# sergree/matchering

Measured on NVIDIA H100. Metric: stereo 44.1kHz samples/sec (x real-time), higher is better.
Workload: dtype f32

## Files before the change

matchering_b200/csrc/limiter.cu:

```cuda
#include <math.h>
#include <string.h>

#include "kernels.cuh"

namespace mgb {

namespace {

constexpr int NT = kLimiterThreads;
constexpr int CORE_EPT = kLimiterCoreEpt;
constexpr int LC = kLimiterCore;
constexpr int SPAN_EPT_MAX = kLimiterSpanEptMax;

__device__ __forceinline__ double scan_carry(double B, const ScanPow* t, double c0, double* scratch) {
    const int lane = threadIdx.x & 31, warp = threadIdx.x >> 5;
    double v = B;
#pragma unroll
    for (int d = 1; d < 32; d <<= 1) {
        const double up = __shfl_up_sync(0xffffffffu, v, d);
        if (lane >= d) v += t->ql[d] * up;
    }
    if (lane == 31) scratch[warp] = v;
    __syncthreads();
    double w = lane < NT / 32 ? scratch[lane] : 0.0;
#pragma unroll
    for (int d = 1; d < NT / 32; d <<= 1) {
        const double up = __shfl_up_sync(0xffffffffu, w, d);
        if (lane >= d) w += t->qw[d] * up;
    }
    const double warp_carry = __shfl_sync(0xffffffffu, w, (warp + 31) & 31);
    double prev = __shfl_up_sync(0xffffffffu, v, 1);
    if (lane == 0) prev = 0.0;
    return prev + t->ql[lane] * ((warp > 0 ? warp_carry : 0.0) + t->qw[warp] * c0);
}

__device__ __forceinline__ double scan_carry_rev(double B, const ScanPow* t, const double* c0, double* scratch) {
    const int lane = threadIdx.x & 31, warp = threadIdx.x >> 5;
    const int rl = 31 - lane, rw = NT / 32 - 1 - warp;
    double v = B;
#pragma unroll
    for (int d = 1; d < 32; d <<= 1) {
        const double up = __shfl_down_sync(0xffffffffu, v, d);
        if (rl >= d) v += t->ql[d] * up;
    }
    if (lane == 0) scratch[rw] = v;
    __syncthreads();
    double w = lane < NT / 32 ? scratch[lane] : 0.0;
#pragma unroll
    for (int d = 1; d < NT / 32; d <<= 1) {
        const double up = __shfl_up_sync(0xffffffffu, w, d);
        if (lane >= d) w += t->qw[d] * up;
    }
    const double warp_carry = __shfl_sync(0xffffffffu, w, (rw + 31) & 31);
    double prev = __shfl_down_sync(0xffffffffu, v, 1);
    if (rl == 0) prev = 0.0;
    return prev + t->ql[rl] * ((rw > 0 ? warp_carry : 0.0) + t->qw[rw] * (*c0));
}

template <int N>
struct StVec {
    double v[N];
};
template <int N>
__device__ __forceinline__ StVec<N> st_zero() {
    StVec<N> z;
#pragma unroll
    for (int i = 0; i < N; ++i) z.v[i] = 0.0;
    return z;
}
template <int N>
__device__ __forceinline__ StVec<N> st_shfl_up(StVec<N> a, int d) {
#pragma unroll
    for (int i = 0; i < N; ++i) a.v[i] = __shfl_up_sync(0xffffffffu, a.v[i], d);
    return a;
}
template <int N>
__device__ __forceinline__ StVec<N> st_shfl(StVec<N> a, int src) {
#pragma unroll
    for (int i = 0; i < N; ++i) a.v[i] = __shfl_sync(0xffffffffu, a.v[i], src);
    return a;
}
template <int N>
__device__ __forceinline__ void st_addmul(StVec<N>& y, const double (*M)[N], const StVec<N>& x) {
#pragma unroll
    for (int r = 0; r < N; ++r)
#pragma unroll
        for (int c = 0; c < N; ++c) y.v[r] += M[r][c] * x.v[c];
}
template <int N>
__device__ __forceinline__ StVec<N> st_mul(const double (*M)[N], const StVec<N>& x) {
    StVec<N> y = st_zero<N>();
    st_addmul<N>(y, M, x);
    return y;
}

template <int N>
__device__ __forceinline__ StVec<N> section_scan(StVec<N> B, const SectionTab<N>* t, double* scratch) {
    const int lane = threadIdx.x & 31, warp = threadIdx.x >> 5;
    StVec<N> v = B;
#pragma unroll
    for (int d = 1; d < 32; d <<= 1) {
        const StVec<N> up = st_shfl_up<N>(v, d);
        if (lane >= d) st_addmul<N>(v, t->ql[d], up);
    }
    if (lane == 31) {
#pragma unroll
        for (int i = 0; i < N; ++i) scratch[warp * N + i] = v.v[i];
    }
    __syncthreads();
    StVec<N> w = st_zero<N>();
    if (lane < NT / 32) {
#pragma unroll
        for (int i = 0; i < N; ++i) w.v[i] = scratch[lane * N + i];
    }
#pragma unroll
    for (int d = 1; d < NT / 32; d <<= 1) {
        const StVec<N> up = st_shfl_up<N>(w, d);
        if (lane >= d) st_addmul<N>(w, t->qw[d], up);
    }
    StVec<N> warp_carry = st_shfl<N>(w, (warp + 31) & 31);
    if (warp == 0) warp_carry = st_zero<N>();
    StVec<N> prev = st_shfl_up<N>(v, 1);
    if (lane == 0) prev = st_zero<N>();
    st_addmul<N>(prev, t->ql[lane], warp_carry);
    return prev;
}

template <int N>
__device__ __forceinline__ StVec<N> section_lead(const SectionTab<N>* t, const StVec<N>& cin) {
    const int lane = threadIdx.x & 31, warp = threadIdx.x >> 5;
    return st_mul<N>(t->ql[lane], st_mul<N>(t->qw[warp], cin));
}

__device__ __forceinline__ void publish(LookbackWord* w, double v, int status) {
#ifdef MGB_EMULATE
    w->value = v;
    w->status = status;
#else
    asm volatile("st.global.cg.v2.u64 [%0], {%1, %2};" ::"l"(w), "l"(__double_as_longlong(v)), "l"((long long)status) : "memory");
#endif
}
__device__ __forceinline__ int poll(const LookbackWord* w, double* v) {
#ifdef MGB_EMULATE
    *v = w->value;
    return (int)w->status;
#else
    long long a, b;
    asm volatile("ld.global.cg.v2.u64 {%0, %1}, [%2];" : "=l"(a), "=l"(b) : "l"(w) : "memory");
    *v = __longlong_as_double(a);
    return (int)b;
#endif
}

template <int N>
__device__ __forceinline__ StVec<N> lookback(const LookbackWord* words , int chunk,
                                             const SectionTab<N>* t) {
    constexpr int STRIDE = 2 * N;
    const int lane = threadIdx.x & 31;
    if constexpr (N == 1) {
        double acc1 = 0.0, m1 = 1.0;
        for (int base = chunk - 1; base >= 0 && m1 > 1e-9; base -= 32) {
            const int j = base - lane;
            int st = 2;
            double val = 0.0;
            if (j >= 0) {
                const LookbackWord* w = words + (long long)j * STRIDE;
                while ((st = poll(w, &val)) == 0) __nanosleep(20);
            }
            const unsigned inclusive = __ballot_sync(0xffffffffu, st == 2);
            const int first = inclusive ? __ffs((int)inclusive) - 1 : 32;
            if (lane <= first) acc1 += m1 * t->pc[lane][0][0] * val;
            if (inclusive) break;
            m1 *= t->pc[32][0][0];
        }
        StVec<N> out;
        out.v[0] = warp_sum(acc1);
        return out;
    }
    StVec<N> acc = st_zero<N>();
    double mult[N][N];
    int jump = 0;
    for (int base = chunk - 1; base >= 0; base -= 32, ++jump) {
        if (N > 1 && jump < kLookbackJumps) {
#pragma unroll
            for (int r = 0; r < N; ++r)
#pragma unroll
                for (int c = 0; c < N; ++c) mult[r][c] = t->pj[jump][r][c];
        } else if (jump == 0) {
#pragma unroll
            for (int r = 0; r < N; ++r)
#pragma unroll
                for (int c = 0; c < N; ++c) mult[r][c] = r == c ? 1.0 : 0.0;
        } else {
            double next[N][N];
#pragma unroll
            for (int r = 0; r < N; ++r)
#pragma unroll
                for (int c = 0; c < N; ++c) {
                    double sum = 0.0;
#pragma unroll
                    for (int k = 0; k < N; ++k) sum += mult[r][k] * t->pc[32][k][c];
                    next[r][c] = sum;
                }
#pragma unroll
            for (int r = 0; r < N; ++r)
#pragma unroll
                for (int c = 0; c < N; ++c) mult[r][c] = next[r][c];
        }
        double bound = 0.0;
#pragma unroll
        for (int r = 0; r < N; ++r) {
            double rowsum = 0.0;
#pragma unroll
            for (int c = 0; c < N; ++c) rowsum += fabs(mult[r][c]);
            bound = fmax(bound, rowsum);
        }
        if (bound <= 1e-9) break;
        const int j = base - lane;
        int st = 2;
        StVec<N> val = st_zero<N>();
        if (j >= 0) {
            const LookbackWord* w = words + (long long)j * STRIDE;
            for (;;) {
                st = poll(w, &val.v[0]);
                bool same = st != 0;
#pragma unroll
                for (int i = 1; i < N; ++i) same = same && poll(w + i, &val.v[i]) == st;
                if (same) break;
                __nanosleep(20);
            }
        }
        const unsigned inclusive = __ballot_sync(0xffffffffu, st == 2);
        const int first = inclusive ? __ffs((int)inclusive) - 1 : 32;
        if (lane <= first) st_addmul<N>(acc, mult, st_mul<N>(t->pc[lane], val));
        if (inclusive) break;
    }
#pragma unroll
    for (int i = 0; i < N; ++i) acc.v[i] = warp_sum(acc.v[i]);
    return acc;
}
template <int N>
__device__ __forceinline__ void publish_state(LookbackWord* words, const StVec<N>& s, int status) {
#pragma unroll
    for (int i = 0; i < N; ++i) publish(words + i, s.v[i], status);
}

struct LimiterGeom {
    int reach, hold, warm, left;
    int ept;
    int span;
    int filt;
    int publish_inclusive;
    int shared_core;
    int margin;
    int use_ticket;
};

__global__ void limiter_tables_kernel(mgb_limiter_params lp, int span_ept, unsigned char* tables) {
    const int i = threadIdx.x;
    ScanPow* att = reinterpret_cast<ScanPow*>(tables);
    {
        const double p = lp.attack_c;
        if (i < SPAN_EPT_MAX + 2) att->pe[i] = pow(p, (double)i);
        if (i < 33) att->ql[i] = pow(p, (double)(span_ept * i));
        if (i < 17) att->qw[i] = pow(p, (double)(span_ept * 32 * i));
        if (i < 33) att->pc[i] = pow(p, (double)LC * (double)i);
    }
    SectionTab<1>* sec = reinterpret_cast<SectionTab<1>*>(tables + sizeof(ScanPow));
    for (int f = 0; f < 2; ++f) {
        const double p = f == 0 ? -lp.hold_a[1] : -lp.release_a[1];
        SectionTab<1>* t = sec + f;
        if (i < CORE_EPT) t->pe[i][0] = pow(p, (double)(i + 1));
        if (i < 33) t->ql[i][0][0] = pow(p, (double)(CORE_EPT * i));
        if (i < 17) t->qw[i][0][0] = pow(p, (double)(CORE_EPT * 32 * i));
        if (i < 33) t->pc[i][0][0] = pow(p, (double)LC * (double)i);
        for (int j = i; j < kLookbackJumps; j += blockDim.x) t->pj[j][0][0] = pow(p, (double)LC * 32.0 * (double)j);
    }
}

template <int EPT, int NO, bool GAINS = false>
__global__ void __launch_bounds__(NT, (NO == 1 && EPT <= 17) ? 2 : 1)
limiter_kernel(mgb_limiter_params lp, LimiterGeom gm, const float2* __restrict__ in, float2* __restrict__ out,
               long long frames, const double* __restrict__ pre_gain, const double* __restrict__ post_gain,
               const int* __restrict__ engaged, int* __restrict__ ticket, LookbackWord* __restrict__ slots,
               const unsigned char* __restrict__ tables) {
    constexpr int HC = CORE_EPT + NO;
    constexpr int CAP = EPT * NT;
    MGB_DYN_SMEM(smem);
    double* Fd = reinterpret_cast<double*>(smem);
    float* Aenv = reinterpret_cast<float*>(smem) + CAP;
    float* G = reinterpret_cast<float*>(smem + (size_t)CAP * 8) + gm.margin;
    float* Wk = G + CAP + gm.margin;
    __shared__ float blockmax[NT];
    __shared__ ScanPow pw_att;
    __shared__ SectionTab<1> pw_sec[2];
    __shared__ double scratch_a[32 * NO], scratch_b[32 * NO];
    __shared__ double bcast[2 + 2 * NO];
    __shared__ int chunk_s;
    const ScanPow* pow_att = &pw_att;
    const SectionTab<NO>* sec_global = reinterpret_cast<const SectionTab<NO>*>(tables + sizeof(ScanPow));
    const SectionTab<NO>* tab_hold = NO == 1 ? reinterpret_cast<const SectionTab<NO>*>(&pw_sec[0]) : sec_global;
    const SectionTab<NO>* tab_rel = NO == 1 ? reinterpret_cast<const SectionTab<NO>*>(&pw_sec[1]) : sec_global + 1;

    const int tid = threadIdx.x;
    int chunk = blockIdx.x;
    if (gm.use_ticket) {
        if (tid == 0) chunk_s = atomicAdd(ticket, 1);
        __syncthreads();
        chunk = chunk_s;
    }
    const long long s0 = (long long)chunk * LC;
    const int core_n = (int)((s0 + LC < frames) ? LC : frames - s0);
    const int reach = gm.reach, hold = gm.hold, HL = gm.left, FL = gm.filt;
    const long long ga = s0 - HL - reach;
    const int cidx = HL + reach;
    const int vlo = ga < 0 ? (int)(-ga) : 0;
    const int vhi = (frames - ga < (long long)gm.span) ? (int)(frames - ga) : gm.span;
    const double thr = lp.threshold;

    float2 v[EPT];
    {
        const float2* base = in + ga;
#pragma unroll
        for (int k = 0; k < EPT; ++k) {
            const int i = tid + k * NT;
            v[k] = (i >= vlo && i < vhi) ? __ldg(base + i) : make_float2(0.0f, 0.0f);
        }
    }
    const double pre = pre_gain ? *pre_gain : 1.0;
    const double post = post_gain ? *post_gain : 1.0;
    const double scale = pre * post;
    const bool bypass = engaged && *engaged == 0;
    {
        const double* src = reinterpret_cast<const double*>(tables);
        double* dst = reinterpret_cast<double*>(&pw_att);
        for (int i = tid; i < (int)(sizeof(ScanPow) / sizeof(double)); i += NT) dst[i] = src[i];
        if (NO == 1) {
            src += sizeof(ScanPow) / sizeof(double);
            dst = reinterpret_cast<double*>(pw_sec);
            for (int i = tid; i < (int)(2 * sizeof(SectionTab<1>) / sizeof(double)); i += NT) dst[i] = src[i];
        }
    }
    if (bypass) {
        for (int k = tid; k < core_n; k += NT) {
            const float2 w = in[s0 + k];
            out[s0 + k] = make_float2((float)((double)w.x * pre * post), (float)((double)w.y * pre * post));
        }
        return;
    }
    for (int i = tid; i < gm.margin; i += NT) {
        G[-1 - i] = 0.0f;
        G[CAP + i] = 0.0f;
    }
#pragma unroll
    for (int k = 0; k < EPT; ++k) {
        const double a = (double)fmaxf(fabsf(v[k].x), fabsf(v[k].y)) * pre;
        const double over = a - thr;
        float g = 0.0f;
        if (over > 0.0) g = __fdiv_rn((float)over, (float)a);
        G[tid + k * NT] = g;
    }
    __syncthreads();

    float hc[HC];
    {
        float* PF = reinterpret_cast<float*>(smem);
        float* SF = Wk;
        float x[EPT];
        const int base = tid * EPT;
#pragma unroll
        for (int e = 0; e < EPT; ++e) x[e] = G[base + e];
        float run = 0.0f;
#pragma unroll
        for (int e = 0; e < EPT; ++e) {
            run = fmaxf(run, x[e]);
            PF[base + e] = run;
        }
        blockmax[tid] = run;
        run = 0.0f;
#pragma unroll
        for (int e = EPT - 1; e >= 0; --e) {
            run = fmaxf(run, x[e]);
            SF[base + e] = run;
        }
        __syncthreads();
        auto whole_blocks = [&](int a, int b) -> float {
            float m = 0.0f;
            for (int q = a; q <= b; ++q) m = fmaxf(m, blockmax[q]);
            return m;
        };
        auto window = [&](int l, int r, int br, float pr) -> float {
            const int bl = l / EPT;
            if (bl == br) {
                float m = 0.0f;
                for (int i = l; i <= r; ++i) m = fmaxf(m, G[i]);
                return m;
            }
            float m = fmaxf(SF[l], pr);
            if (br - bl > 1) m = fmaxf(m, whole_blocks(bl + 1, br - 1));
            return m;
        };
        auto gat = [&](int i) -> float { return G[i]; };
        if (gm.shared_core) {
            float la[EPT], rt[EPT];
#pragma unroll
            for (int e = 0; e < EPT - 1; ++e) {
                la[e] = gat(base - reach + e);
                rt[e + 1] = gat(base + reach + 1 + e);
            }
            la[EPT - 1] = rt[0] = 0.0f;
#pragma unroll
            for (int e = EPT - 2; e >= 0; --e) la[e] = fmaxf(la[e], la[e + 1]);
#pragma unroll
            for (int e = 1; e < EPT; ++e) rt[e] = fmaxf(rt[e], rt[e - 1]);
            const int r = min(base + reach, CAP - 1);
            const float core = window(max(base + EPT - 1 - reach, 0), r, r / EPT, PF[r]);
#pragma unroll
            for (int e = 0; e < EPT; ++e) Aenv[base + e] = fmaxf(core, fmaxf(la[e], rt[e]));
        } else {
#pragma unroll
            for (int e = 0; e < EPT; ++e) {
                const int i = base + e;
                const int r = min(i + reach, CAP - 1);
                Aenv[i] = window(max(i - reach, 0), r, r / EPT, PF[r]);
            }
        }
        const int bh = cidx + tid * CORE_EPT - NO;
        if (gm.shared_core) {
            float lh[HC], rh[HC];
#pragma unroll
            for (int e = 0; e < HC - 1; ++e) {
                lh[e] = gat(bh - reach - hold + 1 + e);
                rh[e + 1] = gat(bh + reach + 1 + e);
            }
            lh[HC - 1] = rh[0] = 0.0f;
#pragma unroll
            for (int e = HC - 2; e >= 0; --e) lh[e] = fmaxf(lh[e], lh[e + 1]);
#pragma unroll
            for (int e = 1; e < HC; ++e) rh[e] = fmaxf(rh[e], rh[e - 1]);
            const int r = min(bh + reach, CAP - 1);
            const float core = window(max(bh + HC - reach - hold, 0), r, r / EPT, PF[r]);
#pragma unroll
            for (int e = 0; e < HC; ++e) hc[e] = fmaxf(core, fmaxf(lh[e], rh[e]));
        } else {
#pragma unroll
            for (int e = 0; e < HC; ++e) {
                const int r = min(bh + e + reach, CAP - 1);
                hc[e] = window(max(bh + e - reach - hold + 1, 0), r, r / EPT, PF[r]);
            }
        }
#pragma unroll
        for (int e = 0; e < HC; ++e)
            if (bh + e < vlo) hc[e] = 0.0f;
    }

    LookbackWord* slot_hold = slots + (long long)chunk * (2 * NO);
    LookbackWord* slot_rel = slot_hold + NO;
    double hold_y[CORE_EPT];
    StVec<NO> hold_carry;
    float* Hown = Wk + tid * HC;
    {
#pragma unroll
        for (int e = 0; e < CORE_EPT; ++e) {
            double acc = lp.hold_b[0] * (double)hc[e + NO];
#pragma unroll
            for (int i = 1; i <= NO; ++i) acc += lp.hold_b[i] * (double)hc[e + NO - i];
#pragma unroll
            for (int i = 1; i <= NO; ++i)
                if (e - i >= 0) acc -= lp.hold_a[i] * hold_y[e - i];
            hold_y[e] = acc;
        }
        StVec<NO> end;
#pragma unroll
        for (int i = 0; i < NO; ++i) end.v[i] = hold_y[CORE_EPT - 1 - i];
        hold_carry = section_scan<NO>(end, tab_hold, scratch_a);
        if (tid == NT - 1) {
            st_addmul<NO>(end, tab_hold->ql[1], hold_carry);
            publish_state<NO>(slot_hold, end, 1);
        }
#pragma unroll
        for (int e = 0; e < HC; ++e) Hown[e] = hc[e];
    }

    const double c = lp.attack_c;
    const bool edge_l = vlo > reach, edge_r = vhi < reach + FL;
    if (edge_l || edge_r) {
        const int i0 = vlo, iL = vhi - 1;
        float fix[EPT];
#pragma unroll
        for (int k = 0; k < EPT; ++k) {
            const int i = tid + k * NT;
            fix[k] = Aenv[i];
            if (i < vlo) {
                const int d = (vlo - i < 6) ? vlo - i : 6;
                fix[k] = 2.0f * Aenv[i0] - Aenv[i0 + d];
            } else if (i >= vhi) {
                const int d = (i - iL < 6) ? i - iL : 6;
                fix[k] = 2.0f * Aenv[iL] - Aenv[iL - d];
            }
        }
        __syncthreads();
#pragma unroll
        for (int k = 0; k < EPT; ++k) Aenv[tid + k * NT] = fix[k];
        __syncthreads();
    }
    {
        double y[EPT];
        double acc = 0.0;
#pragma unroll
        for (int e = 0; e < EPT; ++e) {
            acc = (1.0 - c) * (double)Aenv[tid * EPT + e] + c * acc;
            y[e] = acc;
        }
        const double c0 = (double)Aenv[0];
        const double carry = scan_carry(acc, pow_att, c0, scratch_b);
#pragma unroll
        for (int e = 0; e < EPT; ++e) y[e] += pow_att->pe[e + 1] * carry;
        if (edge_r) {
            const int ilast = (int)(frames + 5 - ga);
            if (ilast < CAP - 1) {
#pragma unroll
                for (int e = 0; e < EPT; ++e)
                    if (tid * EPT + e == ilast) bcast[1] = y[e];
                __syncthreads();
                const double held = bcast[1];
#pragma unroll
                for (int e = 0; e < EPT; ++e)
                    if (tid * EPT + e > ilast) y[e] = held;
                __syncthreads();
            }
        }
        if (tid == NT - 1) bcast[1] = y[EPT - 1];
        acc = 0.0;
#pragma unroll
        for (int e = EPT - 1; e >= 0; --e) {
            acc = (1.0 - c) * y[e] + c * acc;
            y[e] = acc;
        }
        const double back = scan_carry_rev(acc, pow_att, &bcast[1], scratch_a);
#pragma unroll
        for (int e = 0; e < EPT; ++e) {
            const int i = tid * EPT + e;
            if (i >= cidx && i < cidx + LC) {
                const float att = (float)(y[e] + pow_att->pe[EPT - e] * back);
                G[i] = GAINS ? att : fmaxf(G[i], att);
            }
        }
    }

    if (tid < 32) {
        const StVec<NO> cin = lookback<NO>(slots, chunk, tab_hold);
        if (tid == 0) {
#pragma unroll
            for (int i = 0; i < NO; ++i) bcast[2 + i] = cin.v[i];
        }
    }
    __syncthreads();
    StVec<NO> hold_prev;
    {
        StVec<NO> cin;
#pragma unroll
        for (int i = 0; i < NO; ++i) cin.v[i] = bcast[2 + i];
        hold_prev = section_lead<NO>(tab_hold, cin);
#pragma unroll
        for (int i = 0; i < NO; ++i) hold_prev.v[i] += hold_carry.v[i];
#pragma unroll
        for (int e = 0; e < CORE_EPT; ++e)
#pragma unroll
            for (int i = 0; i < NO; ++i) hold_y[e] += tab_hold->pe[e][i] * hold_prev.v[i];
        if (tid == NT - 1 && gm.publish_inclusive) {
            StVec<NO> end;
#pragma unroll
            for (int i = 0; i < NO; ++i) end.v[i] = hold_y[CORE_EPT - 1 - i];
            publish_state<NO>(slot_hold, end, 2);
        }
    }

    {
        double rel_y[CORE_EPT];
        double win[HC];
#pragma unroll
        for (int i = 0; i < NO; ++i) win[i] = fmax((double)Hown[i], hold_prev.v[NO - 1 - i]);
#pragma unroll
        for (int e = 0; e < CORE_EPT; ++e) win[NO + e] = fmax((double)Hown[NO + e], hold_y[e]);
#pragma unroll
        for (int e = 0; e < CORE_EPT; ++e) {
            double acc = lp.release_b[0] * win[e + NO];
#pragma unroll
            for (int i = 1; i <= NO; ++i) acc += lp.release_b[i] * win[e + NO - i];
#pragma unroll
            for (int i = 1; i <= NO; ++i)
                if (e - i >= 0) acc -= lp.release_a[i] * rel_y[e - i];
            rel_y[e] = acc;
        }
        StVec<NO> end;
#pragma unroll
        for (int i = 0; i < NO; ++i) end.v[i] = rel_y[CORE_EPT - 1 - i];
        StVec<NO> rel_prev = section_scan<NO>(end, tab_rel, scratch_b);
        if (tid == NT - 1) {
            st_addmul<NO>(end, tab_rel->ql[1], rel_prev);
            publish_state<NO>(slot_rel, end, 1);
        }
        if (tid < 32) {
            const StVec<NO> cr = lookback<NO>(slots + NO, chunk, tab_rel);
            if (tid == 0) {
#pragma unroll
                for (int i = 0; i < NO; ++i) bcast[2 + NO + i] = cr.v[i];
            }
        }
        __syncthreads();
        {
            StVec<NO> cin;
#pragma unroll
            for (int i = 0; i < NO; ++i) cin.v[i] = bcast[2 + NO + i];
            const StVec<NO> lead = section_lead<NO>(tab_rel, cin);
#pragma unroll
            for (int i = 0; i < NO; ++i) rel_prev.v[i] += lead.v[i];
        }
#pragma unroll
        for (int e = 0; e < CORE_EPT; ++e) {
#pragma unroll
            for (int i = 0; i < NO; ++i) rel_y[e] += tab_rel->pe[e][i] * rel_prev.v[i];
            const int i = cidx + tid * CORE_EPT + e;
            const double g_rel = fmax(hold_y[e], rel_y[e]);
            Fd[tid * CORE_EPT + e] = GAINS ? g_rel : 1.0 - fmax((double)G[i], g_rel);
        }
        if (tid == NT - 1 && gm.publish_inclusive) {
#pragma unroll
            for (int i = 0; i < NO; ++i) end.v[i] = rel_y[CORE_EPT - 1 - i];
            publish_state<NO>(slot_rel, end, 2);
        }
    }
    if (GAINS) __syncthreads();
    else __syncwarp();

    {
        const int wbase = (tid >> 5) * (32 * CORE_EPT) + (tid & 31);
        float2 v[CORE_EPT];
#pragma unroll
        for (int q = 0; q < CORE_EPT; ++q) {
            const int k = wbase + q * 32;
            v[q] = k < core_n ? __ldg(in + s0 + k) : make_float2(0.0f, 0.0f);
        }
#pragma unroll
        for (int q = 0; q < CORE_EPT; ++q) {
            const int k = wbase + q * 32;
            if (k < core_n) {
                if (GAINS) {
                    out[s0 + k] = make_float2(G[cidx + k], (float)Fd[k]);
                } else {
                    const double gain = Fd[k] * scale;
                    out[s0 + k] = make_float2((float)((double)v[q].x * gain), (float)((double)v[q].y * gain));
                }
            }
        }
    }
}

__global__ void limiter_engaged_kernel(const float* peak_bits, const double* pre_gain, double threshold, int* engaged) {
    const double pre = pre_gain ? *pre_gain : 1.0;
    const double peak = (double)(*peak_bits) * pre;
    const double r = fmax(peak, threshold) / threshold;
    *engaged = (fabs(r - 1.0) <= 1e-8 + 1e-5 * 1.0) ? 0 : 1;
}

int limiter_order_capacity(const mgb_limiter_params& lp) {
    return (lp.hold_order <= 1 && lp.release_order <= 1) ? 1 : MGB_MAX_FILTER_ORDER;
}

int limiter_geometry(const mgb_limiter_params& lp, LimiterGeom* g) {
    MGB_REQUIRE(lp.reach >= 1 && lp.hold >= 3 && lp.warmup >= 8, MGB_ERR_INVALID, "limiter: bad window sizes");
    MGB_REQUIRE(lp.hold_order >= 1 && lp.hold_order <= MGB_MAX_FILTER_ORDER && lp.release_order >= 1 &&
                    lp.release_order <= MGB_MAX_FILTER_ORDER,
                MGB_ERR_UNSUPPORTED, "limiter: hold / release filter orders %d / %d, kernels exist for 1..%d", lp.hold_order,
                lp.release_order, MGB_MAX_FILTER_ORDER);
    const int no = limiter_order_capacity(lp);
    MGB_REQUIRE(lp.attack_c > 0.0 && lp.attack_c < 1.0, MGB_ERR_INVALID, "limiter: attack pole out of (0,1)");
    MGB_REQUIRE(lp.threshold > 0.0, MGB_ERR_INVALID, "limiter: threshold must be positive");
    g->reach = lp.reach;
    g->hold = lp.hold;
    g->warm = lp.warmup;
    g->left = lp.warmup > lp.hold + no - 1 ? lp.warmup : lp.hold + no - 1;
    g->filt = LC + g->left + g->warm;
    g->span = g->filt + 2 * g->reach;
    int ept = (g->span + NT - 1) / NT;
    if (!(ept & 1)) ept += 1;
    if (ept < 11) ept = 11;
    if (ept < CORE_EPT + no) ept = (CORE_EPT + no) | 1;
    g->ept = ept;
    g->publish_inclusive = g_lookback_inclusive;
    g->use_ticket = g_limiter_ticket;
    g->shared_core = (2 * lp.reach >= ept - 1 && 2 * lp.reach + lp.hold >= CORE_EPT + no) ? 1 : 0;
    g->margin = (lp.reach + lp.hold + ept + no + 3) / 4 * 4;
    MGB_REQUIRE(ept <= SPAN_EPT_MAX, MGB_ERR_UNSUPPORTED,
                "limiter: halo of %d samples exceeds the kernel's span", g->span - LC);
    return MGB_OK;
}

}

struct SectionPowers {
    long double A, B;
    int kind;
    long double r_log, theta, sin_theta;
    long double p1, p2;
    explicit SectionPowers(const double* a) {
        A = -(long double)a[1];
        B = (long double)a[2];
        if (a[2] == 0.0) {
            kind = 0;
            p1 = A;
            return;
        }
        const double hi = a[1] * a[1];
        const double lo = fma(a[1], a[1], -hi);
        const long double disc = ((long double)hi - 4.0L * B) + (long double)lo;
        if (disc < 0) {
            kind = 1;
            r_log = 0.5L * log1pl(B - 1.0L);
            theta = atan2l(sqrtl(-disc), A);
            sin_theta = sinl(theta);
        } else if (disc > 0) {
            kind = 2;
            const long double q = sqrtl(disc);
            p1 = 0.5L * (A + q);
            p2 = 0.5L * (A - q);
        } else {
            kind = 3;
            p1 = 0.5L * A;
        }
    }
    long double U(long long m) const {
        if (m < 0) return 0.0L;
        switch (kind) {
            case 0: return powl(p1, (long double)m);
            case 1: return expl((long double)m * r_log) * sinl((long double)(m + 1) * theta) / sin_theta;
            case 2: return (powl(p1, (long double)(m + 1)) - powl(p2, (long double)(m + 1))) / (p1 - p2);
            default: return (long double)(m + 1) * powl(p1, (long double)m);
        }
    }
    void power(long long m, double (*out)[2]) const {
        if (m == 0) {
            out[0][0] = out[1][1] = 1.0;
            out[0][1] = out[1][0] = 0.0;
            return;
        }
        const long double u0 = U(m), u1 = U(m - 1), u2 = U(m - 2);
        out[0][0] = (double)u0;
        out[0][1] = (double)(-B * u1);
        out[1][0] = (double)u1;
        out[1][1] = (double)(-B * u2);
    }
};

static void fill_section_tables(const double* a, SectionTab<2>* t) {
    const SectionPowers sp(a);
    double m[2][2];
    for (int e = 0; e < CORE_EPT; ++e) {
        sp.power(e + 1, m);
        t->pe[e][0] = m[0][0];
        t->pe[e][1] = m[0][1];
    }
    for (int k = 0; k < 33; ++k) sp.power((long long)CORE_EPT * k, t->ql[k]);
    for (int k = 0; k < 17; ++k) sp.power((long long)CORE_EPT * 32 * k, t->qw[k]);
    for (int k = 0; k < 33; ++k) sp.power((long long)LC * k, t->pc[k]);
    for (int j = 0; j < kLookbackJumps; ++j) sp.power((long long)LC * 32 * j, t->pj[j]);
}

static void fill_attack_tables(double p, int span_ept, ScanPow* t) {
    for (int i = 0; i < SPAN_EPT_MAX + 2; ++i) t->pe[i] = (double)powl((long double)p, (long double)i);
    for (int i = 0; i < 33; ++i) t->ql[i] = (double)powl((long double)p, (long double)(span_ept * i));
    for (int i = 0; i < 17; ++i) t->qw[i] = (double)powl((long double)p, (long double)(span_ept * 32 * i));
    for (int i = 0; i < 33; ++i) t->pc[i] = (double)powl((long double)p, (long double)LC * (long double)i);
}

int64_t limiter_lookback_bytes(int64_t frames, int order_capacity) {
    const int64_t chunks = (frames + LC - 1) / LC;
    return (chunks * 2 * order_capacity * (int64_t)sizeof(LookbackWord) + 255) / 256 * 256;
}
int64_t limiter_lookback_bytes(const mgb_limiter_params& lp, int64_t frames) {
    return limiter_lookback_bytes(frames, limiter_order_capacity(lp));
}

int64_t limiter_tables_bytes() { return (int64_t)(sizeof(ScanPow) + 2 * sizeof(SectionTab<MGB_MAX_FILTER_ORDER>) + 255) / 256 * 256; }

int launch_limiter_tables(const mgb_limiter_params& lp, void* tables, cudaStream_t stream) {
    LimiterGeom g;
    MGB_TRY(limiter_geometry(lp, &g));
    if (limiter_order_capacity(lp) == 1)
        return launch("limiter_tables_kernel", limiter_tables_kernel, dim3(1), dim3(64), 0, stream, lp, g.ept,
                      (unsigned char*)tables);
    struct Block {
        ScanPow attack;
        SectionTab<2> section[2];
    } block;
    static_assert(sizeof(Block) == sizeof(ScanPow) + 2 * sizeof(SectionTab<2>), "table layout");
    fill_attack_tables(lp.attack_c, g.ept, &block.attack);
    fill_section_tables(lp.hold_a, &block.section[0]);
    fill_section_tables(lp.release_a, &block.section[1]);
#ifdef MGB_EMULATE
    (void)stream;
    memcpy(tables, &block, sizeof(block));
#else
    if (cudaMemcpyAsync(tables, &block, sizeof(block), cudaMemcpyHostToDevice, stream) != cudaSuccess) return cuda_status("limiter tables");
#endif
    return MGB_OK;
}

int launch_limiter(const mgb_limiter_params& lp, const float2* in, float2* out, int64_t frames, const double* pre_gain,
                   const double* post_gain, const int* engaged, int* ticket, void* lookback, const void* tables,
                   cudaStream_t stream, bool gains_only) {
    LimiterGeom g;
    MGB_TRY(limiter_geometry(lp, &g));
    MGB_REQUIRE(frames > 6, MGB_ERR_INVALID, "limiter: the input must be longer than filtfilt's padlen (6)");
    MGB_REQUIRE(tables != nullptr, MGB_ERR_INVALID, "limiter: pole tables missing");
    const int64_t chunks = (frames + LC - 1) / LC;
    const size_t smem = (size_t)g.ept * NT * 16 + (size_t)g.margin * 8;
    const int no = limiter_order_capacity(lp);
    if (gains_only) {
        auto go = [&](auto kernel) {
            return launch("limiter_kernel", kernel, dim3((unsigned)chunks), dim3(NT), smem, stream, lp, g, in, out,
                          (long long)frames, pre_gain, post_gain, engaged, ticket, (LookbackWord*)lookback,
                          (const unsigned char*)tables);
        };
        if (no == 1 && g.ept == 11) return go(limiter_kernel<11, 1, true>);
        if (no == 1 && g.ept == 13) return go(limiter_kernel<13, 1, true>);
        if (no == MGB_MAX_FILTER_ORDER && g.ept == 11) return go(limiter_kernel<11, MGB_MAX_FILTER_ORDER, true>);
        set_error("limiter gains (test entry): no kernel for %d span samples per thread at order capacity %d", g.ept, no);
        return MGB_ERR_UNSUPPORTED;
    }
#define MGB_LIMITER_CASE(E)                                                                                           \
    case E:                                                                                                           \
        if (no == 1)                                                                                                  \
            return launch("limiter_kernel", limiter_kernel<E, 1>, dim3((unsigned)chunks), dim3(NT), smem, stream, lp, g, in, \
                          out, (long long)frames, pre_gain, post_gain, engaged, ticket, (LookbackWord*)lookback,     \
                          (const unsigned char*)tables);                                                             \
        return launch("limiter_kernel", limiter_kernel<E, MGB_MAX_FILTER_ORDER>, dim3((unsigned)chunks), dim3(NT), smem, \
                      stream, lp, g, in, out, (long long)frames, pre_gain, post_gain, engaged, ticket,               \
                      (LookbackWord*)lookback, (const unsigned char*)tables);
    switch (g.ept) {
        MGB_LIMITER_CASE(11)
        MGB_LIMITER_CASE(13)
        MGB_LIMITER_CASE(15)
        MGB_LIMITER_CASE(17)
        MGB_LIMITER_CASE(19)
        MGB_LIMITER_CASE(21)
        MGB_LIMITER_CASE(23)
        MGB_LIMITER_CASE(25)
        default: break;
    }
#undef MGB_LIMITER_CASE
    set_error("limiter: no kernel for %d span samples per thread", g.ept);
    return MGB_ERR_UNSUPPORTED;
}

int launch_limiter_engaged(const float* peak_bits, const double* pre_gain, double threshold, int* engaged,
                           cudaStream_t stream) {
    return launch("limiter_engaged_kernel", limiter_engaged_kernel, dim3(1), dim3(1), 0, stream, peak_bits, pre_gain,
                  threshold, engaged);
}

}
```

Measured before the change: 553,600.

## Fuse forward/backward attack scans and recompute hold filter to cut register pressure

For interior chunks, the attack smoothing now runs its forward and backward exponential scans together in one fused block scan that shares a single barrier, instead of two separate passes. The hold IIR output is no longer kept in registers across the attack phase; it is recomputed from the stored hold input in shared memory once the lookback carry is known. This lowers register pressure and barrier count at the cost of some redundant arithmetic. Optional clock64 phase markers are also added behind a compile flag for profiling.

```diff
diff --git a/matchering_b200/csrc/limiter.cu b/matchering_b200/csrc/limiter.cu
--- a/matchering_b200/csrc/limiter.cu
+++ b/matchering_b200/csrc/limiter.cu
@@ -12,6 +12,15 @@
 constexpr int LC = kLimiterCore;
 constexpr int SPAN_EPT_MAX = kLimiterSpanEptMax;
 
+#ifdef MGB_LIMITER_PHASE_CLOCKS
+constexpr int kPhaseClockChunks = 1 << 16;
+__device__ long long g_phase_clock[kPhaseClockChunks][8];
+#define MGB_PHASE_MARK(p) \
+    if (threadIdx.x == 0 && chunk < kPhaseClockChunks) g_phase_clock[chunk][p] = clock64()
+#else
+#define MGB_PHASE_MARK(p)
+#endif
+
 __device__ __forceinline__ double scan_carry(double B, const ScanPow* t, double c0, double* scratch) {
     const int lane = threadIdx.x & 31, warp = threadIdx.x >> 5;
     double v = B;
@@ -55,6 +64,39 @@
     double prev = __shfl_down_sync(0xffffffffu, v, 1);
     if (rl == 0) prev = 0.0;
     return prev + t->ql[rl] * ((rw > 0 ? warp_carry : 0.0) + t->qw[rw] * (*c0));
+}
+
+__device__ __forceinline__ double2 scan_carry_both(double f, double b, const ScanPow* t, double c0f, double c0b,
+                                                   double* scratch) {
+    constexpr int W = NT / 32;
+    static_assert(2 * W <= 32 && (W & (W - 1)) == 0, "both sets of warp totals must fit one warp's segments");
+    const int lane = threadIdx.x & 31, warp = threadIdx.x >> 5;
+    const int rl = 31 - lane, rw = W - 1 - warp;
+#pragma unroll
+    for (int d = 1; d < 32; d <<= 1) {
+        const double uf = __shfl_up_sync(0xffffffffu, f, d);
+        const double ub = __shfl_down_sync(0xffffffffu, b, d);
+        if (lane >= d) f += t->ql[d] * uf;
+        if (rl >= d) b += t->ql[d] * ub;
+    }
+    if (lane == 31) scratch[warp] = f;
+    if (lane == 0) scratch[W + rw] = b;
+    __syncthreads();
+    double w = lane < 2 * W ? scratch[lane] : 0.0;
+    const int seg = lane & (W - 1);
+#pragma unroll
+    for (int d = 1; d < W; d <<= 1) {
+        const double up = __shfl_up_sync(0xffffffffu, w, d);
+        if (seg >= d) w += t->qw[d] * up;
+    }
+    const double carry_f = __shfl_sync(0xffffffffu, w, (warp + 31) & 31);
+    const double carry_b = __shfl_sync(0xffffffffu, w, W + ((rw + W - 1) & (W - 1)));
+    double prev_f = __shfl_up_sync(0xffffffffu, f, 1);
+    double prev_b = __shfl_down_sync(0xffffffffu, b, 1);
+    if (lane == 0) prev_f = 0.0;
+    if (rl == 0) prev_b = 0.0;
+    return make_double2(prev_f + t->ql[lane] * ((warp > 0 ? carry_f : 0.0) + t->qw[warp] * c0f),
+                        prev_b + t->ql[rl] * ((rw > 0 ? carry_b : 0.0) + t->qw[rw] * c0b));
 }
 
 template <int N>
@@ -309,6 +351,7 @@
         __syncthreads();
         chunk = chunk_s;
     }
+    MGB_PHASE_MARK(0);
     const long long s0 = (long long)chunk * LC;
     const int core_n = (int)((s0 + LC < frames) ? LC : frames - s0);
     const int reach = gm.reach, hold = gm.hold, HL = gm.left, FL = gm.filt;
@@ -361,6 +404,7 @@
         G[tid + k * NT] = g;
     }
     __syncthreads();
+    MGB_PHASE_MARK(1);
 
     float hc[HC];
     {
@@ -453,13 +497,14 @@
         for (int e = 0; e < HC; ++e)
             if (bh + e < vlo) hc[e] = 0.0f;
     }
+    MGB_PHASE_MARK(2);
 
     LookbackWord* slot_hold = slots + (long long)chunk * (2 * NO);
     LookbackWord* slot_rel = slot_hold + NO;
-    double hold_y[CORE_EPT];
     StVec<NO> hold_carry;
     float* Hown = Wk + tid * HC;
     {
+        double hold_y[CORE_EPT];
 #pragma unroll
         for (int e = 0; e < CORE_EPT; ++e) {
             double acc = lp.hold_b[0] * (double)hc[e + NO];
@@ -481,6 +526,7 @@
 #pragma unroll
         for (int e = 0; e < HC; ++e) Hown[e] = hc[e];
     }
+    MGB_PHASE_MARK(3);
 
     const double c = lp.attack_c;
     const bool edge_l = vlo > reach, edge_r = vhi < reach + FL;
@@ -504,7 +550,7 @@
         for (int k = 0; k < EPT; ++k) Aenv[tid + k * NT] = fix[k];
         __syncthreads();
     }
-    {
+    if (edge_l || edge_r) {
         double y[EPT];
         double acc = 0.0;
 #pragma unroll
@@ -546,7 +592,37 @@
                 G[i] = GAINS ? att : fmaxf(G[i], att);
             }
         }
-    }
+    } else {
+        const double k1 = 1.0 - c;
+        const float* at = Aenv + tid * EPT;
+        double fwd = 0.0, bwd = 0.0;
+#pragma unroll
+        for (int j = 0; j < EPT; ++j) {
+            fwd = k1 * (double)at[j] + c * fwd;
+            bwd = k1 * (double)at[EPT - 1 - j] + c * bwd;
+        }
+        const double2 carry = scan_carry_both(fwd, bwd, pow_att, (double)Aenv[0], (double)Aenv[CAP - 1], scratch_b);
+        double F[EPT];
+        fwd = carry.x;
+#pragma unroll
+        for (int e = 0; e < EPT; ++e) {
+            fwd = k1 * (double)at[e] + c * fwd;
+            F[e] = fwd;
+        }
+        const double inv = 1.0 / (1.0 + c);
+        bwd = carry.y;
+#pragma unroll
+        for (int e = EPT - 1; e >= 0; --e) {
+            const double x = k1 * (double)at[e];
+            bwd = x + c * bwd;
+            const int i = tid * EPT + e;
+            if (i >= cidx && i < cidx + LC) {
+                const float att = (float)((F[e] + bwd - x) * inv);
+                G[i] = GAINS ? att : fmaxf(G[i], att);
+            }
+        }
+    }
+    MGB_PHASE_MARK(4);
 
     if (tid < 32) {
         const StVec<NO> cin = lookback<NO>(slots, chunk, tab_hold);
@@ -557,6 +633,7 @@
     }
     __syncthreads();
     StVec<NO> hold_prev;
+    double hold_y[CORE_EPT];
     {
         StVec<NO> cin;
 #pragma unroll
@@ -565,9 +642,14 @@
 #pragma unroll
         for (int i = 0; i < NO; ++i) hold_prev.v[i] += hold_carry.v[i];
 #pragma unroll
-        for (int e = 0; e < CORE_EPT; ++e)
-#pragma unroll
-            for (int i = 0; i < NO; ++i) hold_y[e] += tab_hold->pe[e][i] * hold_prev.v[i];
+        for (int e = 0; e < CORE_EPT; ++e) {
+            double acc = lp.hold_b[0] * (double)Hown[e + NO];
+#pragma unroll
+            for (int i = 1; i <= NO; ++i) acc += lp.hold_b[i] * (double)Hown[e + NO - i];
+#pragma unroll
+            for (int i = 1; i <= NO; ++i) acc -= lp.hold_a[i] * (e - i >= 0 ? hold_y[e - i] : hold_prev.v[i - e - 1]);
+            hold_y[e] = acc;
+        }
         if (tid == NT - 1 && gm.publish_inclusive) {
             StVec<NO> end;
 #pragma unroll
@@ -575,6 +657,7 @@
             publish_state<NO>(slot_hold, end, 2);
         }
     }
+    MGB_PHASE_MARK(5);
 
     {
         double rel_y[CORE_EPT];
@@ -633,6 +716,7 @@
     }
     if (GAINS) __syncthreads();
     else __syncwarp();
+    MGB_PHASE_MARK(6);
 
     {
         const int wbase = (tid >> 5) * (32 * CORE_EPT) + (tid & 31);
@@ -655,6 +739,7 @@
             }
         }
     }
+    MGB_PHASE_MARK(7);
 }
 
 __global__ void limiter_engaged_kernel(const float* peak_bits, const double* pre_gain, double threshold, int* engaged) {
@@ -861,3 +946,11 @@
 }
 
 }
+
+#ifdef MGB_LIMITER_PHASE_CLOCKS
+extern "C" int mgb_limiter_phase_clocks(long long* host, int chunks) {
+    if (chunks > mgb::kPhaseClockChunks) chunks = mgb::kPhaseClockChunks;
+    if (cudaMemcpyFromSymbol(host, mgb::g_phase_clock, (size_t)chunks * 8 * sizeof(long long)) != cudaSuccess) return -1;
+    return chunks;
+}
+#endif
```

Result: no change. 562,500, median of 6 (+1.6%).
